# hellosunking/Microcket

Measured on AMD Instinct MI355X. Metric: read-pairs/sec through sam2pairs+dedup (150 bp PE, hg38 names, SAM text resident in HBM), higher is better.
Workload: dtype u8; 1 GPU; C2: 100 M 150 bp PE Micro-C read pairs, hg38, one MI355X -- 100000000 synthetic 150 bp PE read pairs per GPU, hg38 chromosome names, 1 lane(s), unc mode, sam=no, seed 20260105, one step = one pass over the whole resident data set + duplicate marking of the reported pairs on (chr1,pos1,chr2,pos2,strands) + per-chromosome-pair counts; preset=C2, pairs_per_gpu=100000001, sam_bytes_per_gpu=94584442002, block_groups=2097152, blocks=48, parallelism=shard1: independent read-group shards, no data-path collective

## Files before the change

microcket_amd/csrc/mkt_capi.cpp:

```cpp
#include "mkt_ctx.h"

extern "C" {

int mkt_abi_version(void) { return MKT_ABI_VERSION; }

const char* mkt_strerror(int code) {
    switch (code) {
    case MKT_OK: return "ok";
    case MKT_E_ARG: return "bad argument";
    case MKT_E_NO_DEVICE: return "no usable HIP device (this library has no CPU path)";
    case MKT_E_HIP: return "HIP runtime error";
    case MKT_E_NOMEM: return "out of memory";
    case MKT_E_CAPACITY: return "a QNAME group does not fit the block buffer";
    case MKT_E_KERNEL: return "kernel reported an internal error";
    case MKT_E_STATE: return "call order violated";
    case MKT_E_IO: return "temporary file error";
    case MKT_E_FORMAT: return "file refused";
    default: return "unknown error";
    }
}
const char* mkt_last_error(const mkt_ctx* ctx) { return ctx ? ctx->err.c_str() : g_create_error.c_str(); }

int mkt_device_count(void) {
    int n = 0;
// ... 67 lines not shown
    c->dims_probed = true;
    c->halo_widened = 0;
    if (c->cfg == CFG_SMALL || c->p.tiles != MKT_TILES_AUTO) return;
    c->dims = lean_dims(bytes_per_line);
    if (getenv("MKT_DEBUG_SYNC")) fprintf(stderr, "tile geometry: %.1f bytes per line -> tile %u, halos %u / %u\n", bytes_per_line, c->dims.tile, c->dims.hb, c->dims.hf);
}
static bool shrink_dims(mkt_ctx* c) {
    if (c->cfg == CFG_SMALL || c->dims.tile <= 2048u) return false;
    auto f = [](uint32_t x, uint32_t lo) { uint32_t y = ((uint32_t)(x * 0.6) + 15u) & ~15u; return y < lo ? lo : y; };
    c->dims.tile = f(c->dims.tile, 2048u); c->dims.hb = f(c->dims.hb, 256u); c->dims.hf = f(c->dims.hf, 512u);
    return true;
}
static bool widen_halos(mkt_ctx* c) {
    if (c->cfg == CFG_SMALL || c->halo_widened >= 2) return false;
    const TileDims mx = max_dims();
    auto f = [](uint32_t x, uint32_t hi) { uint32_t y = ((uint32_t)(x * 1.5) + 15u) & ~15u; return y > hi ? hi : y; };
    const uint32_t hb = f(c->dims.hb, mx.hb), hf = f(c->dims.hf, mx.hf);
    const uint32_t delta = (hb - c->dims.hb) + (hf - c->dims.hf);
    if (delta == 0 || c->dims.tile < delta + 2048u) return false;
    c->dims.tile -= delta; c->dims.hb = hb; c->dims.hf = hf;
    ++c->halo_widened;
    if (getenv("MKT_DEBUG_SYNC")) fprintf(stderr, "tile geometry: halos widened -> tile %u, halos %u / %u\n", c->dims.tile, c->dims.hb, c->dims.hf);
    return true;
}
static bool adapt_geometry(mkt_ctx* c, const BlockResult& r) {
    if (c->p.tiles != MKT_TILES_AUTO || c->p.ordered) return false;
    if (r.tiles >= 1000 && (uint64_t)r.pad2 * 500 > r.tiles && widen_halos(c)) return true;
    if (r.tiles >= 8 && (uint64_t)(r.pad - r.pad2) * 8 > r.tiles) return shrink_dims(c);
    return false;
}
static double probe_device_lines(mkt_ctx* c, const uint8_t* d_text, size_t n) {
    const size_t look = n < ((size_t)1 << 20) ? n : ((size_t)1 << 20);
    if (!look) return 0;
    if (!c->h_probe && (c->d_probe.alloc(1) != hipSuccess || c->h_probe.alloc(1) != hipSuccess)) return 0;
    if (hipMemsetAsync(c->d_probe, 0, sizeof(unsigned long long), c->stream) != hipSuccess) return 0;
    if (launch_count_newlines(d_text, look, c->d_probe, c->stream) != hipSuccess) return 0;
    if (hipMemcpyAsync(c->h_probe, c->d_probe, sizeof(unsigned long long), hipMemcpyDeviceToHost, c->stream) != hipSuccess) return 0;
    if (hipStreamSynchronize(c->stream) != hipSuccess) return 0;
    return *c->h_probe ? (double)look / (double)*c->h_probe : (double)look;
}
static void smaller_geometry(mkt_ctx* c, const uint8_t* d_text, size_t n) {
    if (c->cfg != CFG_SMALL && d_text) {
        const double avg = probe_device_lines(c, d_text, n);
        const TileDims d = avg > 0 ? lean_dims(avg) : c->dims;
        if (d.tile < c->dims.tile) { c->dims = d; return; }
    }
    if (!shrink_dims(c)) { c->cfg = CFG_SMALL; c->dims = small_dims(); }
}

struct StreamOut { uint8_t* gp; size_t gp_cap; uint8_t* gs; size_t gs_cap; hipEvent_t k0, k1, done; };
static int enqueue_block(mkt_ctx* c, const uint8_t* d_text, size_t n, int cfg, const TileDims& dims, size_t slot, const StreamOut* so = nullptr) {
    if (((uintptr_t)d_text & 15u) != 0) return fail(c, MKT_E_ARG, "block text must be 16-byte aligned");
    if (n >= kMaxBlock) return fail(c, MKT_E_ARG, "block of %zu bytes: must be < 2 GiB - 64 KiB", n);
    const uint32_t ntiles = num_tiles((uint32_t)n, dims.tile);
    BlockWs ws{nullptr, ntiles};
    const size_t ws_bytes = ws.bytes();
    int rc = ensure(c, c->d_ws, ws_bytes, ws_bytes + ws_bytes / 4, true);
    if (rc) return rc;
    ws.base = c->d_ws;
    if ((ntiles + finish_chunk_tiles() - 1) / finish_chunk_tiles() > BlockWs::kScanWords) return fail(c, MKT_E_ARG, "block has too many tiles for the finish scan");
    if ((rc = ensure_dev(c, c->d_pairs, n / 3 + 65536))) return rc;
    if (c->P.write_sam && (rc = ensure_dev(c, c->d_sam, n + n / 4 + 65536))) return rc;
    if (!c->d_sc && (rc = ensure_sc_list(c, 1))) return rc;
    KArgs a;
    memset(&a, 0, sizeof a);
    a.text = d_text; a.n = (uint32_t)n; a.ntiles = ntiles; a.dims = dims; a.P = c->P;
    a.descA = ws.descA(); a.descB = ws.descB(); a.descC = ws.descC();
    a.tile_last = ws.tile_last(); a.tile_groups = ws.tile_groups(); a.defer_list = ws.defer_list();
    a.cur = ws.cur();
    a.ticket = ws.ticket(); a.defer_count = ws.defer_count(); a.fast_ticket = ws.fast_ticket();
    a.last_tile = ws.last_tile(); a.scan_ticket = ws.scan_ticket(); a.scan_desc = ws.scan_desc();
    a.res = ws.res();
    a.ordered = c->p.ordered ? 1 : 0;
    a.run = c->d_run;
    a.nregions = c->p.ordered ? 1 : kMaxRegions;
    const size_t sc_need = (size_t)a.nregions * ((n / 256 / (size_t)a.nregions) * 2 + 1024);
    if ((rc = ensure(c, c->d_sc_tmp, sc_need, sc_need, true))) return rc;
    a.pairs_rcap = (c->d_pairs.cap() / a.nregions) & ~(uint64_t)15;
    a.sam_rcap = c->P.write_sam ? ((c->d_sam.cap() / a.nregions) & ~(uint64_t)15) : 0;
    a.sc_rcap = c->d_sc_tmp.cap() / a.nregions;
    a.out.pairs = c->d_pairs; a.out.pairs_cap = c->d_pairs.cap();
    a.out.sam = c->d_sam; a.out.sam_cap = c->P.write_sam ? c->d_sam.cap() : 0;
    a.out.sc = c->d_sc_tmp; a.out.sc_cap = c->d_sc_tmp.cap();
    a.sc_list = c->d_sc; a.sc_list_cap = c->d_sc.cap();
    if (c->p.extensions & MKT_EXT_KEYS) {
        if (!c->d_chr) { HIPCHK(c, c->d_chr.alloc(1)); HIPCHK(c, hipMemsetAsync(c->d_chr, 0, sizeof(ChrTab), c->stream)); }
        const size_t per = (n / 64 / (size_t)a.nregions) * 2 + 4096, need = per * a.nregions;
        if ((rc = ensure(c, c->d_keys_raw, need, need, true))) return rc;
        const double per_byte = c->key_density > 0 ? (c->key_density * 2 < 1.0 / 64 ? c->key_density * 2 : 1.0 / 64) : 1.0 / 64;
        const size_t want = (size_t)c->acc.emitted + (size_t)((double)(c->bytes_unsynced + n) * per_byte) + 65536;
        if (!c->d_key_list.fits(want)) {
            size_t ncap = c->d_key_list.cap() ? c->d_key_list.cap() * 2 : ((size_t)1 << 22);
            while (ncap < want) ncap *= 2;
            HIPCHK(c, hipStreamSynchronize(c->stream));
            HIPCHK(c, c->d_key_list.regrow_keep(ncap, c->d_key_list.cap()));
        }
        a.keys_rcap = c->d_keys_raw.cap() / a.nregions;
        a.out.keys = c->d_keys_raw; a.out.keys_cap = c->d_keys_raw.cap(); a.out.chr = c->d_chr;
        a.out.key_lanes = (c->p.extensions & MKT_EXT_LANES) ? 1u : 0u;
        a.key_list = c->d_key_list; a.key_list_cap = c->d_key_list.cap();
    }
#if defined(MKT_STAMPS)
    if (!c->d_stamps) { HIPCHK(c, c->d_stamps.alloc(kStampWords)); HIPCHK(c, hipMemset(c->d_stamps, 0, kStampWords * sizeof(unsigned long long))); }
    a.stamps = getenv("MKT_NO_STAMPS") ? nullptr : c->d_stamps;
    { const char* e = getenv("MKT_DEBUG_STOP"); a.debug_stop = e ? atoi(e) : 0; }
#endif
// ... 559 lines not shown
    int rc = mkt_sync(c);
    if (rc) return rc;
    const uint64_t K = total_groups ? total_groups : c->acc.groups;
    unsigned long long logged = 0;
    if (c->acc.sc) {
        if (!c->d_sc_logged) HIPCHK(c, c->d_sc_logged.alloc(1));
        HIPCHK(c, hipMemsetAsync(c->d_sc_logged, 0, sizeof(unsigned long long), c->stream));
        const uint64_t drop_group = c->acc.drops(drop_last != 0) ? c->acc.groups - 1 : ~0ull;
        HIPCHK(c, launch_sc_logged(c->d_sc, c->acc.sc, drop_group, group_offset, K, (uint32_t)c->p.ref_threads, c->d_sc_logged, c->stream));
        HIPCHK(c, hipMemcpyAsync(&logged, c->d_sc_logged, sizeof logged, hipMemcpyDeviceToHost, c->stream));
        HIPCHK(c, hipStreamSynchronize(c->stream));
    }
    RunStats s = c->acc.finish_logged(drop_last != 0, logged);
    memset(st, 0, sizeof *st);
    st->lowMap = s.counters[C_LOWMAP]; st->manyHits = s.counters[C_MANYHITS]; st->unpaired = s.counters[C_UNPAIRED];
    st->selfCircle = s.counters[C_SELFCIRCLE]; st->trans = s.counters[C_TRANS];
    st->cis10K = s.counters[C_CIS10K]; st->cis1K = s.counters[C_CIS1K]; st->cis0 = s.counters[C_CIS0];
    st->selfCircle_all = s.selfcircle_all;
    st->groups = s.groups; st->pairs = s.pairs; st->pair_bytes = s.pair_bytes; st->sam_bytes = s.sam_bytes;
    st->bytes_in = c->bytes_in; st->blocks = c->blocks;
    {
        std::lock_guard<std::mutex> g(c->mu);
        if (!c->finished) {
            if (!drop_last && (!c->tail_pairs.empty() || !c->tail_sam.empty())) {
                mkt_ctx::Chunk t;
                t.own_pairs.swap(c->tail_pairs); t.own_sam.swap(c->tail_sam);
                c->ready.push_back(std::move(t));
            }
            c->tail_pairs.clear(); c->tail_sam.clear();
            c->finished = true;
        }
    }
    c->cv.notify_all();
    return MKT_OK;
}

int mkt_reset(mkt_ctx* c) {
    if (!c) return MKT_E_ARG;
    HIPCHK(c, hipSetDevice(c->p.device));
    {
        std::unique_lock<std::mutex> lk(c->mu);
        c->cv.wait(lk, [&] { return c->async_rc != MKT_OK || c->jobs.empty(); });
        (void)sync_all(c);
        c->jobs.clear(); c->ready.clear(); c->handed = mkt_ctx::Chunk(); c->handed_valid = false;
        for (int i = 0; i < mkt_ctx::kIn; ++i) c->in[i].busy = false;
        for (int i = 0; i < mkt_ctx::kOut; ++i) { c->outs[i].dev_busy = false; c->outs[i].host_busy = false; }
        c->async_rc = MKT_OK; c->cur = 0; c->seq = 0; c->consumer_async = false;
    }
    HIPCHK(c, hipStreamSynchronize(c->stream));
    fold_timing(c);
    HIPCHK(c, hipMemsetAsync(c->d_run, 0, sizeof(DevRun), c->stream));
    HIPCHK(c, hipStreamSynchronize(c->stream));
    c->acc = RunAccum();
    c->sc_unfolded = 0; c->bytes_unsynced = 0; c->emitted_unfolded = 0;
    c->sc_density = 0; c->key_density = 0; c->probing = true;
    c->dims_probed = c->p.tiles != MKT_TILES_AUTO || c->p.ordered || c->cfg == CFG_SMALL;
    if (c->d_chr) HIPCHK(c, hipMemsetAsync(c->d_chr, 0, sizeof(ChrTab), c->stream));
    c->res_used = c->res_folded = 0;
    c->h_len = 0;
    c->tail_pairs.clear(); c->tail_sam.clear(); c->drained_pairs.clear(); c->drained_sam.clear();
    c->input_done = c->finished = false;
    c->bytes_in = 0; c->blocks = 0;
    return MKT_OK;
}

int mkt_format_log(const mkt_stats* st, char* out, size_t cap) {
    if (!st || !out) return MKT_E_ARG;
    return snprintf(out, cap, "lowMap\t%u\nmanyHits\t%u\nunpaired\t%u\nselfCircle\t%u\ntrans\t%u\ncis10K\t%u\ncis1K\t%u\ncis0\t%u\n",
                    st->lowMap, st->manyHits, st->unpaired, st->selfCircle, st->trans, st->cis10K, st->cis1K, st->cis0);
}

int mkt_get_timing(const mkt_ctx* c, mkt_timing* t) {
    if (!c || !t) return MKT_E_ARG;
    t->tile_kernel_ms = c->folded_ms; t->tile_launches = c->folded_launches; t->tile_bytes = c->folded_bytes; t->other_ms = 0;
    t->tiles = c->tiles_total; t->deferred_tiles = c->tiles_deferred;
    return MKT_OK;
}
int mkt_reset_timing(mkt_ctx* c) {
    if (!c) return MKT_E_ARG;
    c->folded_ms = 0; c->folded_launches = 0; c->folded_bytes = 0; c->tiles_total = 0; c->tiles_deferred = 0;
    std::lock_guard<std::mutex> g(c->mu);
    c->replays = mkt_replays{0, 0, 0, 0, 0};
    return MKT_OK;
}
int mkt_get_replays(const mkt_ctx* c, mkt_replays* r) {
    if (!c || !r) return MKT_E_ARG;
    std::lock_guard<std::mutex> g(const_cast<mkt_ctx*>(c)->mu);
    *r = c->replays;
    return MKT_OK;
}

}
```

microcket_amd/csrc/mkt_capi_ext.cpp:

```cpp
#include "mkt_ctx.h"

extern "C" {

static int ensure_dedup_work(mkt_ctx* c, uint64_t n);
int mkt_ext_dedup(mkt_ctx* c, int drop_last, uint64_t* total, uint64_t* dups, uint8_t* flags, size_t flags_cap) {
    if (!c) return MKT_E_ARG;
    if (!(c->p.extensions & MKT_EXT_KEYS)) return fail(c, MKT_E_STATE, "context created without MKT_EXT_KEYS");
    int rc = mkt_sync(c);
    if (rc) return rc;
    const uint64_t n = ext_key_count(c, drop_last);
    if (total) *total = n;
    if (dups) *dups = 0;
    if (n == 0) return MKT_OK;
    if (flags && flags_cap < n) return fail(c, MKT_E_ARG, "flags buffer too small (%llu needed)", (unsigned long long)n);
    const size_t wb = dedup_work_bytes(n);
    if ((rc = ensure_dedup_work(c, n))) return rc;
    HIPCHK(c, launch_dedup(c->d_key_list, n, c->d_dd_flags, c->d_dd_work.get(), wb, c->d_dd_res, c->stream));
    HIPCHK(c, hipMemcpyAsync(c->h_dd_res, c->d_dd_res, sizeof(DedupResult), hipMemcpyDeviceToHost, c->stream));
    if (flags) HIPCHK(c, hipMemcpyAsync(flags, c->d_dd_flags, n, hipMemcpyDeviceToHost, c->stream));
    HIPCHK(c, hipStreamSynchronize(c->stream));
    if (dups) *dups = c->h_dd_res->dups;
    return MKT_OK;
}
int mkt_ext_chr_names(mkt_ctx* c, char* out, size_t cap, size_t* len) {
    if (!c || !len) return MKT_E_ARG;
    if (!(c->p.extensions & MKT_EXT_KEYS)) return fail(c, MKT_E_STATE, "context created without MKT_EXT_KEYS");
    int rc = mkt_sync(c);
    if (rc) return rc;
    *len = 0;
    if (!c->d_chr) return MKT_OK;
    std::vector<unsigned long long> hh(kChrSlots);
    std::vector<uint8_t> names((size_t)kChrSlots * 64);
    HIPCHK(c, hipMemcpy(hh.data(), c->d_chr->hash, kChrSlots * sizeof(unsigned long long), hipMemcpyDeviceToHost));
    HIPCHK(c, hipMemcpy(names.data(), c->d_chr->name, names.size(), hipMemcpyDeviceToHost));
    std::string txt;
    char num[16];
    for (uint32_t s2 = 0; s2 < kChrSlots; ++s2) if (hh[s2]) {
        snprintf(num, sizeof num, "%u", s2);
        txt += num; txt += '\t'; txt.append((const char*)&names[(size_t)s2 * 64], names[(size_t)s2 * 64 + 63]); txt += '\n';
    }
    *len = txt.size();
    if (out) { if (cap < txt.size()) return fail(c, MKT_E_ARG, "buffer too small (%zu needed)", txt.size()); memcpy(out, txt.data(), txt.size()); }
    return MKT_OK;
}
int mkt_ext_keys_fetch(mkt_ctx* c, int drop_last, void* keys, size_t cap_bytes, uint64_t* n) {
    if (!c || !n) return MKT_E_ARG;
    if (!(c->p.extensions & MKT_EXT_KEYS)) return fail(c, MKT_E_STATE, "context created without MKT_EXT_KEYS");
    int rc = mkt_sync(c);
    if (rc) return rc;
    *n = ext_key_count(c, drop_last);
    if (keys && *n) {
        if (cap_bytes < *n * sizeof(KeyRec)) return fail(c, MKT_E_ARG, "key buffer too small (%llu bytes needed)", (unsigned long long)(*n * sizeof(KeyRec)));
        HIPCHK(c, hipMemcpy(keys, c->d_key_list, (size_t)*n * sizeof(KeyRec), hipMemcpyDeviceToHost));
    }
    return MKT_OK;
}
static int ensure_dedup_work(mkt_ctx* c, uint64_t n) {
    const size_t wb = dedup_work_bytes(n);
    int rc;
    if ((rc = ensure(c, c->d_dd_flags, n, n + n / 8 + 4096, false))) return rc;
    if ((rc = ensure(c, c->d_dd_work, wb, wb + wb / 8, false))) return rc;
    if (!c->h_dd_res) { HIPCHK(c, c->d_dd_res.alloc(1)); HIPCHK(c, c->h_dd_res.alloc(1)); }
    return MKT_OK;
}
int mkt_ext_dedup_device(mkt_ctx* c, const void* d_keys, uint64_t n, uint8_t* d_flags, uint64_t* dups) {
    if (!c || (n && (!d_keys || !d_flags))) return MKT_E_ARG;
    HIPCHK(c, hipSetDevice(c->p.device));
    if (dups) *dups = 0;
    if (n == 0) return MKT_OK;
    int rc = ensure_dedup_work(c, n);
    if (rc) return rc;
    HIPCHK(c, launch_dedup((const KeyRec*)d_keys, n, d_flags, c->d_dd_work.get(), dedup_work_bytes(n), c->d_dd_res, c->stream));
    HIPCHK(c, hipMemcpyAsync(c->h_dd_res, c->d_dd_res, sizeof(DedupResult), hipMemcpyDeviceToHost, c->stream));
    HIPCHK(c, hipStreamSynchronize(c->stream));
// ... 129 lines not shown
                    const hipError_t e = hipDeviceEnablePeerAccess(cs[b]->p.device, 0);
                    if (e != hipSuccess) (void)hipGetLastError();
                }
            }
    for (uint32_t r = 0; r < world; ++r) {
        mkt_ctx* c = cs[r];
        HIPCHK(c, hipSetDevice(c->p.device));
        sd[r].nrecv = 0;
        for (uint32_t s2 = 0; s2 < world; ++s2) sd[r].nrecv += sd[s2].cnt[r];
        if (!sd[r].nrecv) continue;
        HIPCHK(c, sd[r].d_recv.alloc((size_t)sd[r].nrecv * sizeof(KeyRec)));
        HIPCHK(c, sd[r].d_flags.alloc((size_t)sd[r].nrecv));
        uint64_t at = 0;
        for (uint32_t s2 = 0; s2 < world; ++s2) {
            uint64_t soff = 0;
            for (uint32_t d = 0; d < r; ++d) soff += sd[s2].cnt[d];
            const uint64_t k = sd[s2].cnt[r];
            if (k) HIPCHK(c, hipMemcpyPeerAsync(sd[r].d_recv + at * sizeof(KeyRec), c->p.device, sd[s2].d_send + soff * sizeof(KeyRec), cs[s2]->p.device, (size_t)k * sizeof(KeyRec), c->stream));
            at += k;
        }
    }
    uint64_t all_dups = 0;
    for (uint32_t r = 0; r < world; ++r) {
        mkt_ctx* c = cs[r];
        HIPCHK(c, hipSetDevice(c->p.device));
        HIPCHK(c, hipStreamSynchronize(c->stream));
        uint64_t d = 0;
        const int rc = mkt_ext_dedup_device(c, sd[r].d_recv, sd[r].nrecv, sd[r].d_flags, &d);
        if (rc) return rc;
        all_dups += d;
    }
    for (uint32_t s2 = 0; s2 < world; ++s2) {
        mkt_ctx* c = cs[s2];
        HIPCHK(c, hipSetDevice(c->p.device));
        if (!sd[s2].n) { dups[s2] = 0; continue; }
        HIPCHK(c, sd[s2].d_back.alloc((size_t)sd[s2].n));
        uint64_t soff = 0;
        for (uint32_t r = 0; r < world; ++r) {
            uint64_t roff = 0;
            for (uint32_t q = 0; q < s2; ++q) roff += sd[q].cnt[r];
            const uint64_t k = sd[s2].cnt[r];
            if (k) HIPCHK(c, hipMemcpyPeerAsync(sd[s2].d_back + soff, c->p.device, sd[r].d_flags + roff, cs[r]->p.device, (size_t)k, c->stream));
            soff += k;
        }
        HIPCHK(c, hipStreamSynchronize(c->stream));
        const int rc = mkt_ext_unpartition(c, sd[s2].d_back, flags ? flags[s2] : nullptr, flags_cap ? flags_cap[s2] : 0, &dups[s2]);
        if (rc) return rc;
    }
    uint64_t sum = 0;
    for (uint32_t r = 0; r < world; ++r) sum += dups[r];
    if (sum != all_dups) return fail(c0, MKT_E_KERNEL, "duplicate counts disagree after the exchange (%llu marked, %llu returned)", (unsigned long long)all_dups, (unsigned long long)sum);
    return MKT_OK;
}
int mkt_ext_chrstat(mkt_ctx* c, int drop_last, char* out, size_t cap, size_t* len) {
    if (!c || !len) return MKT_E_ARG;
    if (!(c->p.extensions & MKT_EXT_KEYS)) return fail(c, MKT_E_STATE, "context created without MKT_EXT_KEYS");
    int rc = mkt_sync(c);
    if (rc) return rc;
    *len = 0;
    const uint64_t n = ext_key_count(c, drop_last);
    if (n == 0 || !c->d_chr) return MKT_OK;
    const size_t name_bytes = (size_t)kChrSlots * 64, hash_bytes = kChrSlots * sizeof(unsigned long long);
    if (!c->h_chr_stage) HIPCHK(c, c->h_chr_stage.alloc(hash_bytes + name_bytes + kChrSlots * sizeof(uint16_t)));
    unsigned long long* hh = (unsigned long long*)c->h_chr_stage.get();
    uint8_t* names = c->h_chr_stage + hash_bytes;
    uint16_t* dense = (uint16_t*)(c->h_chr_stage + hash_bytes + name_bytes);
    HIPCHK(c, hipMemcpyAsync(hh, c->d_chr->hash, hash_bytes, hipMemcpyDeviceToHost, c->stream));
    HIPCHK(c, hipMemcpyAsync(names, c->d_chr->name, name_bytes, hipMemcpyDeviceToHost, c->stream));
    HIPCHK(c, hipStreamSynchronize(c->stream));
    std::vector<std::pair<std::string, uint32_t>> used;
    for (uint32_t s2 = 0; s2 < kChrSlots; ++s2) if (hh[s2]) used.emplace_back(std::string((const char*)&names[(size_t)s2 * 64], names[(size_t)s2 * 64 + 63]), s2);
    std::sort(used.begin(), used.end());
    const uint32_t nd = (uint32_t)used.size();
    memset(dense, 0, kChrSlots * sizeof(uint16_t));
    for (uint32_t d = 0; d < nd; ++d) dense[used[d].second] = (uint16_t)d;
    const size_t cells = (size_t)nd * nd, cnt_bytes = cells * sizeof(unsigned long long);
    if (!c->d_dense) HIPCHK(c, c->d_dense.alloc(kChrSlots));
    if ((rc = ensure(c, c->d_chr_counts, cells, cells, false)) || (rc = ensure(c, c->h_chr_counts, cells, cells, false))) return rc;
    HIPCHK(c, hipMemcpyAsync(c->d_dense, dense, kChrSlots * sizeof(uint16_t), hipMemcpyHostToDevice, c->stream));
    HIPCHK(c, hipMemsetAsync(c->d_chr_counts, 0, cnt_bytes, c->stream));
    HIPCHK(c, launch_chrstat(c->d_key_list, n, c->d_dense, nd, c->d_chr_counts, c->stream));
    HIPCHK(c, hipMemcpyAsync(c->h_chr_counts, c->d_chr_counts, cnt_bytes, hipMemcpyDeviceToHost, c->stream));
    HIPCHK(c, hipStreamSynchronize(c->stream));
    const unsigned long long* counts = c->h_chr_counts;
    std::string txt;
    char num[32];
    for (uint32_t a2 = 0; a2 < nd; ++a2)
        for (uint32_t b2 = 0; b2 < nd; ++b2)
            if (counts[(size_t)a2 * nd + b2]) {
                snprintf(num, sizeof num, "%llu", counts[(size_t)a2 * nd + b2]);
                txt += used[a2].first; txt += '\t'; txt += used[b2].first; txt += '\t'; txt += num; txt += '\n';
            }
    *len = txt.size();
    if (out) { if (cap < txt.size()) return fail(c, MKT_E_ARG, "chrstat buffer too small (%zu needed)", txt.size()); memcpy(out, txt.data(), txt.size()); }
    return MKT_OK;
}

}
```

microcket_amd/csrc/mkt_ctx.h:

```cpp
#pragma once
#include <hip/hip_runtime.h>
#include <stdarg.h>
#include <stdio.h>
#include <stdlib.h>
#include <string.h>
#include <algorithm>
#include <string>
#include <utility>
#include <chrono>
#include <condition_variable>
#include <deque>
#include <mutex>
#include <thread>
#include <vector>

#include "../../include/mkt.h"
#include "mkt_launch.h"
#include "mkt_devbuf.h"

using namespace mkt;

static const size_t kMaxBlock = ((size_t)1 << 31) - 65536;
static const uint32_t kFastRoundsDefault = 8;
static const size_t kStampWords = 20;

inline thread_local std::string g_create_error;

struct mkt_ctx {
    mkt_params p;
    Params P;
    DevStream stream, s_in, s_out;
    int cfg = CFG_FAST;
    TileDims dims = {0, 0, 0};
    bool dims_probed = false;
    DevBuf<unsigned long long> d_probe; PinBuf<unsigned long long> h_probe;
    TileDims last_dims = {0, 0, 0};
    const uint8_t* last_text = nullptr;
    bool probing = true;
    size_t block_cap = 0;
    GrowBuf<uint8_t> d_pairs, d_sam;
    GrowBuf<uint64_t> d_sc;
    DevBuf<unsigned long long> d_sc_logged;
    PinBuf<uint8_t> h_chr_stage; DevBuf<uint16_t> d_dense;
    GrowBuf<uint8_t> d_dd_flags, d_dd_work;
    DevBuf<DedupResult> d_dd_res; PinBuf<DedupResult> h_dd_res;
    GrowBuf<uint32_t> d_perm; DevBuf<uint32_t> d_part_hist; DevBuf<uint16_t> d_lut; uint64_t part_n = 0;
    GrowBuf<unsigned long long> d_chr_counts; PinGrowBuf<unsigned long long> h_chr_counts;
    double sc_density = 0;
    GrowBuf<uint64_t> d_sc_tmp;
    GrowBuf<KeyRec> d_keys_raw;
    GrowBuf<KeyRec> d_key_list;
    DevBuf<ChrTab> d_chr;
    GrowBuf<uint8_t> d_ws;
    DevBuf<DevRun> d_run;
    size_t h_len = 0;
    PinBuf<BlockResult> h_res; size_t res_slots = 0, res_used = 0, res_folded = 0;
    std::vector<DevBuf<uint8_t>> uploads;
    std::vector<const uint8_t*> res_text; std::vector<size_t> res_n;
    static constexpr int kIn = 3, kOut = 2;
    static constexpr size_t kHead = 65536;
    enum { EV_H2D, EV_K0, EV_K1, EV_DONE };
    struct InSlot { PinBuf<uint8_t> h; DevBuf<uint8_t> d; bool busy = false; DevEvents<4> ev; };
    struct OutSlot { GrowBuf<uint8_t> d_pairs, d_sam; PinGrowBuf<uint8_t> h; bool dev_busy = false, host_busy = false; };
    struct Job { int in_slot, out_slot; size_t n; int cfg; TileDims dims; int attempts; };
    struct Chunk { const char* pairs = nullptr; size_t pairs_len = 0; const char* sam = nullptr; size_t sam_len = 0; int out_slot = -1;
                   std::vector<char> own_pairs, own_sam; };
    InSlot in[kIn];
    OutSlot outs[kOut];
    std::deque<Job> jobs;
    std::deque<Chunk> ready;
    Chunk handed; bool handed_valid = false;
    std::mutex mu;
    std::condition_variable cv;
    std::thread worker;
    bool worker_started = false, stop = false;
    int async_rc = MKT_OK;
    bool consumer_async = false;
    int cur = 0;
    uint64_t seq = 0;
    std::vector<char> tail_pairs, tail_sam, drained_pairs, drained_sam;
    RunAccum acc;
    bool input_done = false, finished = false;
    uint64_t bytes_in = 0, blocks = 0;
    size_t last_n = 0;
    double key_density = 0;
    uint64_t emitted_unfolded = 0;
    uint64_t sc_unfolded = 0;
    uint64_t bytes_unsynced = 0;
    struct Timed { DevEvents<2> ev; uint64_t bytes = 0; };
    std::deque<Timed> ev;
    double folded_ms = 0; uint64_t folded_launches = 0, folded_bytes = 0;
    uint64_t tiles_total = 0, tiles_deferred = 0;
    mkt_replays replays = {0, 0, 0, 0, 0};
    GrowBuf<char> d_syn;
    GrowBuf<uint64_t> d_syn_sizes;
    DevBuf<unsigned long long> d_stamps;
    uint32_t fast_rounds = kFastRoundsDefault;
    bool no_lean = false;
    int halo_widened = 0;
    std::string err;
// ... 36 lines not shown
```

microcket_amd/csrc/mkt_kernels.hip:

```cpp
#include <hip/hip_runtime.h>
#include <type_traits>
#include "mkt_launch.h"

namespace mkt {

constexpr int NT = 256;
constexpr uint64_t FLAG_AGG = 1ull << 62, FLAG_PREFIX = 2ull << 62, PAYLOAD = (1ull << 62) - 1;
constexpr uint32_t LOOKBACK_SPIN_LIMIT = 1u << 22;

struct ScanScratch { uint64_t a[NT / 64], b[NT / 64]; };

#if defined(MKT_STAMPS)
#define STAMP_DECL() unsigned long long stamp_prev_ = 0, stamp_first_ = 0, stamp_acc_[16] = {0, 0, 0, 0, 0, 0, 0, 0, 0, 0, 0, 0, 0, 0, 0, 0}
#define STAMP(k)                                                                        \
    do {                                                                                \
        if (tid == 0 && a.stamps) {                                                     \
            const unsigned long long now_ = __builtin_amdgcn_s_memtime();               \
            if ((k) > 0) stamp_acc_[(k)] += now_ - stamp_prev_;                         \
            else if (!stamp_first_) stamp_first_ = __builtin_amdgcn_s_memrealtime();   \
            stamp_prev_ = now_;                                                         \
        }                                                                               \
    } while (0)
#define STAMP_SPAN(t0_)                                                                 \
    do {                                                                                \
// ... 1026 lines not shown

uint32_t fast_max_workgroups(int) { return 256u * 4u; }

hipError_t launch_tiles(const KArgs& a, int cfg, int grid, hipStream_t s) {
    if (a.ntiles == 0) return hipSuccess;
    if (!dims_ok(a.dims, cfg == CFG_SMALL ? small_dims() : max_dims())) return hipErrorInvalidValue;
    if (cfg == CFG_SMALL) hipLaunchKernelGGL(k_tiles<CfgSmall>, dim3(grid), dim3(NT), 0, s, a);
    else hipLaunchKernelGGL(k_tiles<CfgFast>, dim3(grid), dim3(NT), 0, s, a);
    return hipGetLastError();
}
hipError_t launch_fast(const KArgs& a, int, int grid, hipStream_t s) {
    if (a.ntiles == 0) return hipSuccess;
    if (!dims_ok(a.dims, max_dims())) return hipErrorInvalidValue;
    hipLaunchKernelGGL((k_fast<CfgLean, NT, 2, 4>), dim3(grid), dim3(NT), 0, s, a);
    return hipGetLastError();
}
__global__ void k_count_nl(const uint8_t* text, size_t n, unsigned long long* out) {
    unsigned long long mine = 0;
    const size_t nv = n >> 4;
    for (size_t v = (size_t)blockIdx.x * blockDim.x + threadIdx.x; v < nv; v += (size_t)gridDim.x * blockDim.x) {
        const uint4 x = reinterpret_cast<const uint4*>(text)[v];
        mine += __popc(nl_flags(x.x)) + __popc(nl_flags(x.y)) + __popc(nl_flags(x.z)) + __popc(nl_flags(x.w));
    }
    if (blockIdx.x == 0 && threadIdx.x == 0) for (size_t b = nv << 4; b < n; ++b) mine += text[b] == '\n';
    for (int d = 32; d >= 1; d >>= 1) mine += shfl_xor64(mine, d);
    if ((threadIdx.x & 63) == 0 && mine) atomicAdd(out, mine);
}
hipError_t launch_count_newlines(const uint8_t* text, size_t n, unsigned long long* out, hipStream_t s) {
    if (n) hipLaunchKernelGGL(k_count_nl, dim3(64), dim3(256), 0, s, text, n, out);
    return hipGetLastError();
}
hipError_t launch_finish(const KArgs& a, hipStream_t s) {
    const unsigned chunks = (a.ntiles + NTF - 1) / NTF;
    if (chunks) hipLaunchKernelGGL(k_finish_scan, dim3(chunks), dim3(NTF), 0, s, a);
    hipLaunchKernelGGL(k_finish, dim3(kFinishGrid), dim3(NTF), 0, s, a);
    if (a.keys_rcap) hipLaunchKernelGGL(k_keys_place, dim3(2048), dim3(256), 0, s, a);
    hipLaunchKernelGGL(k_run_advance, dim3(1), dim3(64), 0, s, a);
    return hipGetLastError();
}
uint32_t finish_chunk_tiles() { return NTF; }

constexpr int DD_WG = 256;
constexpr int DS_WG = 512;
constexpr int DS_NW = DS_WG / 64;
constexpr int DS_T = 8192;
constexpr int DS_K = DS_T / DS_WG;
constexpr int DS_D = 7, DS_R = 1 << DS_D;
constexpr int DS_SCAN_WG = 1024, DS_SCAN_V = 8;
constexpr uint64_t kKeyMask1 = 0xFFFFFFFFC000FFFFull;
static_assert(DS_R == 2 * 64, "the scatter's prologue gives each lane of wave 0 two digits");

__device__ inline bool key_eq(const KeyRec& x, const KeyRec& y) { return x.k0 == y.k0 && (x.k1 & kKeyMask1) == (y.k1 & kKeyMask1); }

__global__ __launch_bounds__(DS_WG) void k_dd_prep(const KeyRec* keys, uint64_t n, int ib, uint64_t* rec, uint32_t* cnt, uint32_t G) {
    __shared__ uint32_t c[DS_R];
    if (threadIdx.x < DS_R) c[threadIdx.x] = 0;
    __syncthreads();
    const uint64_t b = (uint64_t)blockIdx.x * DS_T, e = b + DS_T < n ? b + DS_T : n, hi = ~((1ull << ib) - 1ull);
    for (uint64_t j = b + threadIdx.x; j < e; j += DS_WG) {
        const uint64_t r = (mix64(keys[j].k0 ^ mix64(keys[j].k1 & kKeyMask1)) & hi) | j;
        rec[j] = r;
        atomicAdd(&c[(r >> ib) & (DS_R - 1)], 1u);
    }
    __syncthreads();
    if (threadIdx.x < DS_R) cnt[threadIdx.x * G + blockIdx.x] = c[threadIdx.x];
}
__global__ __launch_bounds__(DS_WG) void k_dd_count(const uint64_t* rec, uint64_t n, int shift, uint32_t* cnt, uint32_t G) {
    __shared__ uint32_t c[DS_R];
    if (threadIdx.x < DS_R) c[threadIdx.x] = 0;
    __syncthreads();
    const uint64_t b = (uint64_t)blockIdx.x * DS_T, m = (b + DS_T < n ? b + DS_T : n) - b;
    const ulonglong2* v = reinterpret_cast<const ulonglong2*>(rec + b);
    for (uint64_t i = threadIdx.x; i < m / 2; i += DS_WG) {
        const ulonglong2 x = v[i];
        atomicAdd(&c[(x.x >> shift) & (DS_R - 1)], 1u);
        atomicAdd(&c[(x.y >> shift) & (DS_R - 1)], 1u);
    }
    if ((m & 1) && threadIdx.x == 0) atomicAdd(&c[(rec[b + m - 1] >> shift) & (DS_R - 1)], 1u);
    __syncthreads();
    if (threadIdx.x < DS_R) cnt[threadIdx.x * G + blockIdx.x] = c[threadIdx.x];
}
__global__ __launch_bounds__(DS_SCAN_WG) void k_dd_dscan(uint32_t* cnt, uint32_t G, uint32_t* tot) {
    __shared__ uint32_t wsum[DS_SCAN_WG / 64];
    const int lane = threadIdx.x & 63, wv = threadIdx.x >> 6;
    uint32_t* row = cnt + (uint64_t)blockIdx.x * G;
    uint32_t carry = 0;
    for (uint32_t base = 0; base < G; base += DS_SCAN_WG * DS_SCAN_V) {
        const uint32_t i0 = base + threadIdx.x * DS_SCAN_V;
        uint32_t v[DS_SCAN_V], s = 0;
#pragma unroll
        for (int k = 0; k < DS_SCAN_V; ++k) { v[k] = i0 + k < G ? row[i0 + k] : 0u; s += v[k]; }
        const uint32_t inc = wave_iscan32(s);
        if (lane == 63) wsum[wv] = inc;
        __syncthreads();
        uint32_t pre = carry, all = 0;
#pragma unroll
        for (int w = 0; w < DS_SCAN_WG / 64; ++w) { const uint32_t x = wsum[w]; if (w < wv) pre += x; all += x; }
        pre += inc - s;
#pragma unroll
        for (int k = 0; k < DS_SCAN_V; ++k) { if (i0 + k < G) row[i0 + k] = pre; pre += v[k]; }
        carry += all;
        __syncthreads();
    }
    if (threadIdx.x == 0) tot[blockIdx.x] = carry;
}
__global__ __launch_bounds__(DS_WG, 4) void k_dd_scatter(const uint64_t* rec, uint64_t n, int shift, const uint32_t* cnt, const uint32_t* tot, uint32_t G, uint64_t* rec2) {
    __shared__ uint64_t tile[DS_T];
    __shared__ uint32_t wrun[DS_NW][DS_R];
    __shared__ uint32_t gdelta[DS_R];
    const int tid = threadIdx.x, lane = tid & 63, wv = tid >> 6;
    const uint64_t b = (uint64_t)blockIdx.x * DS_T, m = (b + DS_T < n ? b + DS_T : n) - b;
    uint32_t gc0 = 0, gc1 = 0, t0 = 0, t1 = 0;
    if (wv == 0) {
        gc0 = cnt[(uint64_t)(2 * lane) * G + blockIdx.x]; gc1 = cnt[(uint64_t)(2 * lane + 1) * G + blockIdx.x];
        t0 = tot[2 * lane]; t1 = tot[2 * lane + 1];
    }
    for (int i = tid; i < DS_NW * DS_R; i += DS_WG) (&wrun[0][0])[i] = 0u;
    __syncthreads();
// ... 38 lines not shown
    __syncthreads();
#pragma unroll
    for (int k = 0; k < DS_K; ++k) {
        const uint64_t i = (uint64_t)wv * (DS_T / DS_NW) + k * 64 + lane;
        if (i < m) tile[wrun[wv][(uint32_t)(r[k] >> shift) & (DS_R - 1)] + ((loc[k / 2] >> (16 * (k & 1))) & 0xFFFFu)] = r[k];
    }
    __syncthreads();
    for (uint32_t i = tid; i < m; i += DS_WG) {
        const uint64_t x = tile[i];
        rec2[gdelta[(uint32_t)(x >> shift) & (DS_R - 1)] + i] = x;
    }
}
__global__ __launch_bounds__(NT) void k_dd_scan(uint32_t* hist, uint32_t m) {
    __shared__ ScanScratch sc;
    __shared__ uint64_t carry;
    if (threadIdx.x == 0) carry = 0;
    __syncthreads();
    for (uint32_t base = 0; base < m; base += NT) {
        const uint32_t i = base + threadIdx.x;
        uint64_t x = i < m ? hist[i] : 0, d = 0, tx, td, e = x;
        block_exscan2(e, d, tx, td, sc);
        if (i < m) hist[i] = (uint32_t)(carry + e);
        __syncthreads();
        if (threadIdx.x == 0) carry += tx;
        __syncthreads();
    }
}
__global__ __launch_bounds__(256) void k_dd_mark(const KeyRec* keys, const uint64_t* rec, uint64_t n, int ib, uint64_t run_mask, uint8_t* flags, DedupResult* res) {
    const uint64_t imask = (1ull << ib) - 1ull, j = (uint64_t)blockIdx.x * blockDim.x + threadIdx.x;
    bool dup = false;
    if (j < n) {
        const uint64_t r = rec[j];
        uint64_t o = j ? rec[j - 1] : ~r;
        bool have = false;
        KeyRec me;
        for (uint64_t b = j - 1; !((o ^ r) & run_mask);) {
            if (!((o ^ r) >> ib)) {
                if (!have) { me = keys[r & imask]; have = true; }
                if (key_eq(keys[o & imask], me)) { dup = true; break; }
            }
            if (b-- == 0) break;
            o = rec[b];
        }
        if (dup) flags[r & imask] = 1;
    }
    const uint64_t m = __ballot(dup);
    if ((threadIdx.x & 63) == 0 && m) atomicAdd((unsigned long long*)&res->dups, (unsigned long long)__popcll(m));
    if (blockIdx.x == 0 && threadIdx.x == 0) res->total = n;
}
size_t dedup_work_bytes(uint64_t n) {
    const uint64_t G = (n + DS_T - 1) / DS_T;
    return (size_t)(n * (8 + 8) + DS_R * (G + 1) * 4 + 4096);
}
hipError_t launch_dedup(const KeyRec* keys, uint64_t n, uint8_t* flags, void* work, size_t work_bytes, DedupResult* d_res, hipStream_t s) {
    hipError_t e = hipMemsetAsync(d_res, 0, sizeof(DedupResult), s);
    if (e != hipSuccess || n == 0) return e;
    if (work_bytes < dedup_work_bytes(n) || n >= (1ull << 32)) return hipErrorInvalidValue;
    const uint32_t G = (uint32_t)((n + DS_T - 1) / DS_T);
    uint8_t* w = (uint8_t*)(((uintptr_t)work + 255) & ~(uintptr_t)255);
    uint64_t* rA = (uint64_t*)w; w += ((n * 8 + 255) & ~255ull);
    uint64_t* rB = (uint64_t*)w; w += ((n * 8 + 255) & ~255ull);
    uint32_t* cnt = (uint32_t*)w;
    uint32_t* tot = cnt + (uint64_t)DS_R * G;
    int ib = 1;
    while ((1ull << ib) < n) ++ib;
    int bits = 2;
    while (bits < 34 && (1ull << (bits - 2)) < n) ++bits;
    bits = bits < 12 ? 12 : (bits > 32 ? 32 : bits);
    const int passes = (bits + DS_D - 1) / DS_D;
    const int sorted = passes * DS_D < 64 - ib ? passes * DS_D : 64 - ib;
    hipLaunchKernelGGL(k_dd_prep, dim3(G), dim3(DS_WG), 0, s, keys, n, ib, rA, cnt, G);
    for (int p = 0; p < passes; ++p) {
        if (p) hipLaunchKernelGGL(k_dd_count, dim3(G), dim3(DS_WG), 0, s, (const uint64_t*)rA, n, ib + DS_D * p, cnt, G);
        hipLaunchKernelGGL(k_dd_dscan, dim3(DS_R), dim3(DS_SCAN_WG), 0, s, cnt, G, tot);
        hipLaunchKernelGGL(k_dd_scatter, dim3(G), dim3(DS_WG), 0, s, (const uint64_t*)rA, n, ib + DS_D * p, (const uint32_t*)cnt, (const uint32_t*)tot, G, rB);
        uint64_t* t = rA; rA = rB; rB = t;
    }
    const uint64_t run_mask = ((1ull << sorted) - 1ull) << ib;
    e = hipMemsetAsync(flags, 0, n, s);
    if (e != hipSuccess) return e;
    hipLaunchKernelGGL(k_dd_mark, dim3((unsigned)((n + 255) / 256)), dim3(256), 0, s, keys, (const uint64_t*)rA, n, ib, run_mask, flags, d_res);
    return hipGetLastError();
}
size_t radix64_count_bytes(uint64_t n) { return (size_t)(DS_R * ((n + DS_T - 1) / DS_T + 1) * 4 + 4096); }
hipError_t launch_radix64(uint64_t*& rA, uint64_t*& rB, uint64_t n, int lo_bit, int nbits, uint32_t* cnt, hipStream_t s) {
    if (n == 0 || nbits <= 0) return hipSuccess;
    if (n >= (1ull << 32) || lo_bit < 0 || lo_bit + nbits > 64) return hipErrorInvalidValue;
    const uint32_t G = (uint32_t)((n + DS_T - 1) / DS_T);
    uint32_t* tot = cnt + (uint64_t)DS_R * G;
    for (int sh = lo_bit; sh < lo_bit + nbits; sh += DS_D) {
        hipLaunchKernelGGL(k_dd_count, dim3(G), dim3(DS_WG), 0, s, (const uint64_t*)rA, n, sh, cnt, G);
        hipLaunchKernelGGL(k_dd_dscan, dim3(DS_R), dim3(DS_SCAN_WG), 0, s, cnt, G, tot);
        hipLaunchKernelGGL(k_dd_scatter, dim3(G), dim3(DS_WG), 0, s, (const uint64_t*)rA, n, sh, (const uint32_t*)cnt, (const uint32_t*)tot, G, rB);
        uint64_t* t = rA; rA = rB; rB = t;
    }
    return hipGetLastError();
}

constexpr uint32_t kMaxWorld = 16;
__device__ inline KeyRec part_remap(KeyRec r, const uint16_t* lut) {
    if (lut) {
        const uint64_t a = lut[(r.k0 >> 45) & (kChrSlots - 1u)], b = lut[(r.k0 >> 32) & (kChrSlots - 1u)];
        r.k0 = (a << 45) | (b << 32) | (r.k0 & 0xFFFFFFFFull);
    }
    return r;
}
__device__ inline uint32_t part_dest(const KeyRec& r, uint32_t world) { return (uint32_t)(mix64(r.k0 ^ mix64(r.k1 & kKeyMask1)) % world); }
__global__ __launch_bounds__(DD_WG) void k_part_hist(const KeyRec* keys, uint64_t n, uint64_t per, const uint16_t* lut, uint32_t world, uint32_t* hist, uint32_t G) {
    __shared__ uint32_t cnt[kMaxWorld];
    if (threadIdx.x < kMaxWorld) cnt[threadIdx.x] = 0;
    __syncthreads();
    const uint64_t b = (uint64_t)blockIdx.x * per, e = b + per < n ? b + per : n;
    for (uint64_t j = b + threadIdx.x; j < e; j += DD_WG) atomicAdd(&cnt[part_dest(part_remap(keys[j], lut), world)], 1u);
    __syncthreads();
    if (threadIdx.x < kMaxWorld) hist[threadIdx.x * G + blockIdx.x] = cnt[threadIdx.x];
}
__global__ __launch_bounds__(DD_WG) void k_part_scatter(const KeyRec* keys, uint64_t n, uint64_t per, const uint16_t* lut, uint32_t world, const uint32_t* hist,
                                                       uint32_t G, KeyRec* send, uint32_t* perm) {
    __shared__ uint32_t base[kMaxWorld];
    __shared__ uint32_t wcnt[DD_WG / 64][kMaxWorld];
    const int tid = threadIdx.x, lane = tid & 63, wv = tid >> 6;
    if (tid < (int)kMaxWorld) base[tid] = hist[tid * G + blockIdx.x];
    __syncthreads();
    const uint64_t b = (uint64_t)blockIdx.x * per, e = b + per < n ? b + per : n;
// ... 175 lines not shown
```

microcket_amd/csrc/mkt_launch.h:

```cpp
#pragma once
#include <hip/hip_runtime.h>
#include "mkt_host.h"
#include "mkt_fast.h"
#include "mkt_synth.h"

namespace mkt {

enum { CFG_FAST = 0, CFG_SMALL = 1 };

struct DevRun { uint64_t groups, sc, emitted; };

struct alignas(128) RegionCur { unsigned long long a, b; unsigned long long pad[14]; };
constexpr int kMaxRegions = 16;
constexpr int kCurShift = 36;
constexpr unsigned long long kCurLow = (1ull << kCurShift) - 1ull;

constexpr uint32_t kFastAllStatic = 0xFFFFFFFFu;
struct KArgs {
    const uint8_t* text;
    uint32_t n;
    uint32_t ntiles;
    TileDims dims;
    uint32_t fast_dyn0;
    Params P;
// ... 13 lines not shown
    int32_t use_list;
    BlockResult* res;
    DevRun* run;
    RegionCur* cur;
    int32_t nregions;
    uint64_t pairs_rcap, sam_rcap, sc_rcap;
    uint64_t* sc_list;
    uint64_t sc_list_cap;
    uint64_t keys_rcap;
    KeyRec* key_list;
    uint64_t key_list_cap;
    OutPtrs out;
    unsigned long long* stamps;
    int32_t debug_stop;
};

struct BlockWs {
    uint8_t* base;
    uint32_t ntiles;
    static constexpr size_t kScanWords = 1024;
    size_t tiles_bytes() const { return ((size_t)ntiles * (3 * sizeof(uint64_t) + sizeof(TileLast) + sizeof(uint64_t) + sizeof(uint32_t)) + 127) & ~(size_t)127; }
    size_t bytes() const { return tiles_bytes() + kMaxRegions * sizeof(RegionCur) + 256 + kScanWords * sizeof(uint64_t) + sizeof(BlockResult); }
    uint64_t* descA() const { return (uint64_t*)base; }
    uint64_t* descB() const { return descA() + ntiles; }
    uint64_t* descC() const { return descB() + ntiles; }
    TileLast* tile_last() const { return (TileLast*)(descC() + ntiles); }
    uint64_t* tile_groups() const { return (uint64_t*)(tile_last() + ntiles); }
    uint32_t* defer_list() const { return (uint32_t*)(tile_groups() + ntiles); }
    RegionCur* cur() const { return (RegionCur*)(base + tiles_bytes()); }
    uint8_t* counters() const { return (uint8_t*)(cur() + kMaxRegions); }
    uint32_t* ticket() const { return (uint32_t*)counters(); }
    uint32_t* defer_count() const { return (uint32_t*)(counters() + 64); }
    uint32_t* defer_ticket() const { return (uint32_t*)(counters() + 128); }
    uint32_t* fast_ticket() const { return (uint32_t*)(counters() + 160); }
    int* last_tile() const { return (int*)(counters() + 192); }
    uint32_t* scan_ticket() const { return (uint32_t*)(counters() + 224); }
    uint64_t* scan_desc() const { return (uint64_t*)(counters() + 256); }
    BlockResult* res() const { return (BlockResult*)(scan_desc() + kScanWords); }
};

TileDims small_dims();
TileDims max_dims();
uint32_t fast_max_workgroups(int cfg);
hipError_t launch_count_newlines(const uint8_t* text, size_t n, unsigned long long* out, hipStream_t s);
hipError_t launch_tiles(const KArgs& a, int cfg, int grid, hipStream_t s);
hipError_t launch_fast(const KArgs& a, int cfg, int grid, hipStream_t s);
uint32_t finish_chunk_tiles();
hipError_t launch_finish(const KArgs& a, hipStream_t s);
hipError_t launch_gather(const BlockResult* d_res, const uint8_t* src, uint64_t rcap, uint8_t* dst, uint64_t dst_cap, int which, uint64_t max_bytes, hipStream_t s);
hipError_t launch_sc_logged(const uint64_t* list, uint64_t n, uint64_t drop_group, uint64_t group_offset, uint64_t K_total, uint32_t ref_threads,
                            unsigned long long* out, hipStream_t s);

struct DedupResult { uint64_t total, dups; };
hipError_t launch_dedup(const KeyRec* keys, uint64_t n, uint8_t* flags, void* work, size_t work_bytes, DedupResult* d_res, hipStream_t s);
size_t dedup_work_bytes(uint64_t n);
size_t radix64_count_bytes(uint64_t n);
hipError_t launch_radix64(uint64_t*& rA, uint64_t*& rB, uint64_t n, int lo_bit, int nbits, uint32_t* cnt, hipStream_t s);
size_t partition_work_bytes();
hipError_t launch_partition(const KeyRec* keys, uint64_t n, const uint16_t* d_lut, uint32_t world, uint32_t* hist, KeyRec* send, uint32_t* perm, uint32_t* G_out, hipStream_t s);
hipError_t launch_unpermute(const uint8_t* in, const uint32_t* perm, uint64_t n, uint8_t* out, unsigned long long* dups, hipStream_t s);
hipError_t launch_chrstat(const KeyRec* keys, uint64_t n, const uint16_t* dense_of_slot, uint32_t ndense, unsigned long long* counts, hipStream_t s);

hipError_t launch_synth_sizes(const SynParams& p, uint64_t first, uint64_t n, uint64_t* sizes, hipStream_t s);
hipError_t launch_exscan(uint64_t* v, uint64_t n, uint64_t* total, hipStream_t s);
hipError_t launch_synth_write(const SynParams& p, uint64_t first, uint64_t n, const uint64_t* offs, char* out, hipStream_t s);
hipError_t launch_synth_tail(const SynParams& p, char* out, hipStream_t s);
size_t synth_tail_bytes(const SynParams& p);

}
```

Before: 2.339 billion read-pairs/s.

## Fuse per-chromosome-pair counting into dedup prep kernel and stash results

The chromosome-pair count histogram is now computed inside the dedup prep kernel, which already reads every key. Counts go to a shared-memory 32x32 table, with global atomics as the fallback. The result is stashed on the host and validated by a generation counter, key count and emitted count, so the later chrstat call skips its own pass over the keys and its separate kernel launch. The trade-off is a grid-stride prep kernel capped at 2048 workgroups, an extra host sync for the dense map before dedup, and stash invalidation logic that must stay correct.

```diff
diff --git a/microcket_amd/csrc/mkt_capi.cpp b/microcket_amd/csrc/mkt_capi.cpp
--- a/microcket_amd/csrc/mkt_capi.cpp
+++ b/microcket_amd/csrc/mkt_capi.cpp
@@ -143,6 +143,7 @@
 static int enqueue_block(mkt_ctx* c, const uint8_t* d_text, size_t n, int cfg, const TileDims& dims, size_t slot, const StreamOut* so = nullptr) {
     if (((uintptr_t)d_text & 15u) != 0) return fail(c, MKT_E_ARG, "block text must be 16-byte aligned");
     if (n >= kMaxBlock) return fail(c, MKT_E_ARG, "block of %zu bytes: must be < 2 GiB - 64 KiB", n);
+    ++c->key_gen;
     const uint32_t ntiles = num_tiles((uint32_t)n, dims.tile);
     BlockWs ws{nullptr, ntiles};
     const size_t ws_bytes = ws.bytes();
@@ -808,6 +809,7 @@
     HIPCHK(c, hipMemsetAsync(c->d_run, 0, sizeof(DevRun), c->stream));
     HIPCHK(c, hipStreamSynchronize(c->stream));
     c->acc = RunAccum();
+    ++c->key_gen; c->chr_stash.valid = false;
     c->sc_unfolded = 0; c->bytes_unsynced = 0; c->emitted_unfolded = 0;
     c->sc_density = 0; c->key_density = 0; c->probing = true;
     c->dims_probed = c->p.tiles != MKT_TILES_AUTO || c->p.ordered || c->cfg == CFG_SMALL;
diff --git a/microcket_amd/csrc/mkt_capi_ext.cpp b/microcket_amd/csrc/mkt_capi_ext.cpp
--- a/microcket_amd/csrc/mkt_capi_ext.cpp
+++ b/microcket_amd/csrc/mkt_capi_ext.cpp
@@ -3,6 +3,8 @@
 extern "C" {
 
 static int ensure_dedup_work(mkt_ctx* c, uint64_t n);
+typedef std::vector<std::pair<std::string, uint32_t>> ChrNames;
+static int chr_dense_map(mkt_ctx* c, ChrNames& used);
 int mkt_ext_dedup(mkt_ctx* c, int drop_last, uint64_t* total, uint64_t* dups, uint8_t* flags, size_t flags_cap) {
     if (!c) return MKT_E_ARG;
     if (!(c->p.extensions & MKT_EXT_KEYS)) return fail(c, MKT_E_STATE, "context created without MKT_EXT_KEYS");
@@ -15,11 +17,23 @@
     if (flags && flags_cap < n) return fail(c, MKT_E_ARG, "flags buffer too small (%llu needed)", (unsigned long long)n);
     const size_t wb = dedup_work_bytes(n);
     if ((rc = ensure_dedup_work(c, n))) return rc;
-    HIPCHK(c, launch_dedup(c->d_key_list, n, c->d_dd_flags, c->d_dd_work.get(), wb, c->d_dd_res, c->stream));
+    mkt_ctx::ChrStash& st = c->chr_stash;
+    st.valid = false;
+    st.used.clear();
+    if (c->d_chr && (rc = chr_dense_map(c, st.used))) return rc;
+    const uint32_t nd = (uint32_t)st.used.size();
+    const size_t cnt_bytes = (size_t)nd * nd * sizeof(unsigned long long);
+    HIPCHK(c, launch_dedup(c->d_key_list, n, c->d_dd_flags, c->d_dd_work.get(), wb, c->d_dd_res, c->stream,
+                           nd ? c->d_dense.get() : nullptr, nd, nd ? c->d_chr_counts.get() : nullptr));
     HIPCHK(c, hipMemcpyAsync(c->h_dd_res, c->d_dd_res, sizeof(DedupResult), hipMemcpyDeviceToHost, c->stream));
+    if (nd) HIPCHK(c, hipMemcpyAsync(c->h_chr_counts, c->d_chr_counts, cnt_bytes, hipMemcpyDeviceToHost, c->stream));
     if (flags) HIPCHK(c, hipMemcpyAsync(flags, c->d_dd_flags, n, hipMemcpyDeviceToHost, c->stream));
     HIPCHK(c, hipStreamSynchronize(c->stream));
     if (dups) *dups = c->h_dd_res->dups;
+    if (nd) {
+        st.counts.assign(c->h_chr_counts.get(), c->h_chr_counts.get() + (size_t)nd * nd);
+        st.n = n; st.emitted = c->acc.emitted; st.gen = c->key_gen; st.valid = true;
+    }
     return MKT_OK;
 }
 int mkt_ext_chr_names(mkt_ctx* c, char* out, size_t cap, size_t* len) {
@@ -255,14 +269,7 @@
     if (sum != all_dups) return fail(c0, MKT_E_KERNEL, "duplicate counts disagree after the exchange (%llu marked, %llu returned)", (unsigned long long)all_dups, (unsigned long long)sum);
     return MKT_OK;
 }
-int mkt_ext_chrstat(mkt_ctx* c, int drop_last, char* out, size_t cap, size_t* len) {
-    if (!c || !len) return MKT_E_ARG;
-    if (!(c->p.extensions & MKT_EXT_KEYS)) return fail(c, MKT_E_STATE, "context created without MKT_EXT_KEYS");
-    int rc = mkt_sync(c);
-    if (rc) return rc;
-    *len = 0;
-    const uint64_t n = ext_key_count(c, drop_last);
-    if (n == 0 || !c->d_chr) return MKT_OK;
+static int chr_dense_map(mkt_ctx* c, ChrNames& used) {
     const size_t name_bytes = (size_t)kChrSlots * 64, hash_bytes = kChrSlots * sizeof(unsigned long long);
     if (!c->h_chr_stage) HIPCHK(c, c->h_chr_stage.alloc(hash_bytes + name_bytes + kChrSlots * sizeof(uint16_t)));
     unsigned long long* hh = (unsigned long long*)c->h_chr_stage.get();
@@ -271,21 +278,43 @@
     HIPCHK(c, hipMemcpyAsync(hh, c->d_chr->hash, hash_bytes, hipMemcpyDeviceToHost, c->stream));
     HIPCHK(c, hipMemcpyAsync(names, c->d_chr->name, name_bytes, hipMemcpyDeviceToHost, c->stream));
     HIPCHK(c, hipStreamSynchronize(c->stream));
-    std::vector<std::pair<std::string, uint32_t>> used;
+    used.clear();
     for (uint32_t s2 = 0; s2 < kChrSlots; ++s2) if (hh[s2]) used.emplace_back(std::string((const char*)&names[(size_t)s2 * 64], names[(size_t)s2 * 64 + 63]), s2);
     std::sort(used.begin(), used.end());
     const uint32_t nd = (uint32_t)used.size();
+    if (nd == 0) return MKT_OK;
     memset(dense, 0, kChrSlots * sizeof(uint16_t));
     for (uint32_t d = 0; d < nd; ++d) dense[used[d].second] = (uint16_t)d;
-    const size_t cells = (size_t)nd * nd, cnt_bytes = cells * sizeof(unsigned long long);
+    const size_t cells = (size_t)nd * nd;
+    int rc;
     if (!c->d_dense) HIPCHK(c, c->d_dense.alloc(kChrSlots));
     if ((rc = ensure(c, c->d_chr_counts, cells, cells, false)) || (rc = ensure(c, c->h_chr_counts, cells, cells, false))) return rc;
     HIPCHK(c, hipMemcpyAsync(c->d_dense, dense, kChrSlots * sizeof(uint16_t), hipMemcpyHostToDevice, c->stream));
-    HIPCHK(c, hipMemsetAsync(c->d_chr_counts, 0, cnt_bytes, c->stream));
-    HIPCHK(c, launch_chrstat(c->d_key_list, n, c->d_dense, nd, c->d_chr_counts, c->stream));
-    HIPCHK(c, hipMemcpyAsync(c->h_chr_counts, c->d_chr_counts, cnt_bytes, hipMemcpyDeviceToHost, c->stream));
-    HIPCHK(c, hipStreamSynchronize(c->stream));
-    const unsigned long long* counts = c->h_chr_counts;
+    HIPCHK(c, hipMemsetAsync(c->d_chr_counts, 0, cells * sizeof(unsigned long long), c->stream));
+    return MKT_OK;
+}
+int mkt_ext_chrstat(mkt_ctx* c, int drop_last, char* out, size_t cap, size_t* len) {
+    if (!c || !len) return MKT_E_ARG;
+    if (!(c->p.extensions & MKT_EXT_KEYS)) return fail(c, MKT_E_STATE, "context created without MKT_EXT_KEYS");
+    int rc = mkt_sync(c);
+    if (rc) return rc;
+    *len = 0;
+    const uint64_t n = ext_key_count(c, drop_last);
+    if (n == 0 || !c->d_chr) return MKT_OK;
+    const mkt_ctx::ChrStash& st = c->chr_stash;
+    const bool stashed = st.valid && st.n == n && st.emitted == c->acc.emitted && st.gen == c->key_gen;
+    ChrNames mapped;
+    if (!stashed) {
+        if ((rc = chr_dense_map(c, mapped))) return rc;
+        const uint32_t nd0 = (uint32_t)mapped.size();
+        if (nd0 == 0) return MKT_OK;
+        HIPCHK(c, launch_chrstat(c->d_key_list, n, c->d_dense, nd0, c->d_chr_counts, c->stream));
+        HIPCHK(c, hipMemcpyAsync(c->h_chr_counts, c->d_chr_counts, (size_t)nd0 * nd0 * sizeof(unsigned long long), hipMemcpyDeviceToHost, c->stream));
+        HIPCHK(c, hipStreamSynchronize(c->stream));
+    }
+    const ChrNames& used = stashed ? st.used : mapped;
+    const unsigned long long* counts = stashed ? st.counts.data() : c->h_chr_counts.get();
+    const uint32_t nd = (uint32_t)used.size();
     std::string txt;
     char num[32];
     for (uint32_t a2 = 0; a2 < nd; ++a2)
diff --git a/microcket_amd/csrc/mkt_ctx.h b/microcket_amd/csrc/mkt_ctx.h
--- a/microcket_amd/csrc/mkt_ctx.h
+++ b/microcket_amd/csrc/mkt_ctx.h
@@ -46,6 +46,13 @@
     DevBuf<DedupResult> d_dd_res; PinBuf<DedupResult> h_dd_res;
     GrowBuf<uint32_t> d_perm; DevBuf<uint32_t> d_part_hist; DevBuf<uint16_t> d_lut; uint64_t part_n = 0;
     GrowBuf<unsigned long long> d_chr_counts; PinGrowBuf<unsigned long long> h_chr_counts;
+    struct ChrStash {
+        bool valid = false;
+        uint64_t n = 0, emitted = 0, gen = 0;
+        std::vector<std::pair<std::string, uint32_t>> used;
+        std::vector<unsigned long long> counts;
+    } chr_stash;
+    uint64_t key_gen = 0;
     double sc_density = 0;
     GrowBuf<uint64_t> d_sc_tmp;
     GrowBuf<KeyRec> d_keys_raw;
diff --git a/microcket_amd/csrc/mkt_kernels.hip b/microcket_amd/csrc/mkt_kernels.hip
--- a/microcket_amd/csrc/mkt_kernels.hip
+++ b/microcket_amd/csrc/mkt_kernels.hip
@@ -1102,18 +1102,39 @@
 
 __device__ inline bool key_eq(const KeyRec& x, const KeyRec& y) { return x.k0 == y.k0 && (x.k1 & kKeyMask1) == (y.k1 & kKeyMask1); }
 
-__global__ __launch_bounds__(DS_WG) void k_dd_prep(const KeyRec* keys, uint64_t n, int ib, uint64_t* rec, uint32_t* cnt, uint32_t G) {
+constexpr uint32_t kPrepChrGrid = 2048;
+template <bool CHR>
+__global__ __launch_bounds__(DS_WG) void k_dd_prep(const KeyRec* keys, uint64_t n, int ib, uint64_t* rec, uint32_t* cnt, uint32_t G,
+                                                   const uint16_t* dense_of_slot, uint32_t ndense, unsigned long long* chr_counts) {
     __shared__ uint32_t c[DS_R];
-    if (threadIdx.x < DS_R) c[threadIdx.x] = 0;
-    __syncthreads();
-    const uint64_t b = (uint64_t)blockIdx.x * DS_T, e = b + DS_T < n ? b + DS_T : n, hi = ~((1ull << ib) - 1ull);
-    for (uint64_t j = b + threadIdx.x; j < e; j += DS_WG) {
-        const uint64_t r = (mix64(keys[j].k0 ^ mix64(keys[j].k1 & kKeyMask1)) & hi) | j;
-        rec[j] = r;
-        atomicAdd(&c[(r >> ib) & (DS_R - 1)], 1u);
-    }
-    __syncthreads();
-    if (threadIdx.x < DS_R) cnt[threadIdx.x * G + blockIdx.x] = c[threadIdx.x];
+    __shared__ uint32_t loc[CHR ? 32 * 32 : 1];
+    if (CHR) for (int k = threadIdx.x; k < 1024; k += DS_WG) loc[k] = 0;
+    const uint64_t hi = ~((1ull << ib) - 1ull);
+    for (uint32_t t = blockIdx.x; t < G; t += gridDim.x) {
+        if (threadIdx.x < DS_R) c[threadIdx.x] = 0;
+        __syncthreads();
+        const uint64_t b = (uint64_t)t * DS_T, e = b + DS_T < n ? b + DS_T : n;
+        for (uint64_t j = b + threadIdx.x; j < e; j += DS_WG) {
+            const uint64_t k0 = keys[j].k0;
+            const uint64_t r = (mix64(k0 ^ mix64(keys[j].k1 & kKeyMask1)) & hi) | j;
+            rec[j] = r;
+            atomicAdd(&c[(r >> ib) & (DS_R - 1)], 1u);
+            if (CHR) {
+                const uint32_t ca = dense_of_slot[(k0 >> 45) & (kChrSlots - 1u)], cb = dense_of_slot[(k0 >> 32) & (kChrSlots - 1u)];
+                if (ca < 32u && cb < 32u) atomicAdd(&loc[ca * 32u + cb], 1u);
+                else if (ca < ndense && cb < ndense) atomicAdd(&chr_counts[(uint64_t)ca * ndense + cb], 1ull);
+            }
+        }
+        __syncthreads();
+        if (threadIdx.x < DS_R) cnt[threadIdx.x * G + t] = c[threadIdx.x];
+    }
+    if (CHR) {
+        __syncthreads();
+        for (int k = threadIdx.x; k < 1024; k += DS_WG) {
+            const uint32_t ca = k >> 5, cb = k & 31;
+            if (loc[k] && ca < ndense && cb < ndense) atomicAdd(&chr_counts[(uint64_t)ca * ndense + cb], (unsigned long long)loc[k]);
+        }
+    }
 }
 __global__ __launch_bounds__(DS_WG) void k_dd_count(const uint64_t* rec, uint64_t n, int shift, uint32_t* cnt, uint32_t G) {
     __shared__ uint32_t c[DS_R];
@@ -1258,7 +1279,8 @@
     const uint64_t G = (n + DS_T - 1) / DS_T;
     return (size_t)(n * (8 + 8) + DS_R * (G + 1) * 4 + 4096);
 }
-hipError_t launch_dedup(const KeyRec* keys, uint64_t n, uint8_t* flags, void* work, size_t work_bytes, DedupResult* d_res, hipStream_t s) {
+hipError_t launch_dedup(const KeyRec* keys, uint64_t n, uint8_t* flags, void* work, size_t work_bytes, DedupResult* d_res, hipStream_t s,
+                        const uint16_t* dense_of_slot, uint32_t ndense, unsigned long long* chr_counts) {
     hipError_t e = hipMemsetAsync(d_res, 0, sizeof(DedupResult), s);
     if (e != hipSuccess || n == 0) return e;
     if (work_bytes < dedup_work_bytes(n) || n >= (1ull << 32)) return hipErrorInvalidValue;
@@ -1275,7 +1297,10 @@
     bits = bits < 12 ? 12 : (bits > 32 ? 32 : bits);
     const int passes = (bits + DS_D - 1) / DS_D;
     const int sorted = passes * DS_D < 64 - ib ? passes * DS_D : 64 - ib;
-    hipLaunchKernelGGL(k_dd_prep, dim3(G), dim3(DS_WG), 0, s, keys, n, ib, rA, cnt, G);
+    if (chr_counts && dense_of_slot && ndense)
+        hipLaunchKernelGGL(k_dd_prep<true>, dim3(G < kPrepChrGrid ? G : kPrepChrGrid), dim3(DS_WG), 0, s, keys, n, ib, rA, cnt, G, dense_of_slot, ndense, chr_counts);
+    else
+        hipLaunchKernelGGL(k_dd_prep<false>, dim3(G), dim3(DS_WG), 0, s, keys, n, ib, rA, cnt, G, (const uint16_t*)nullptr, 0u, (unsigned long long*)nullptr);
     for (int p = 0; p < passes; ++p) {
         if (p) hipLaunchKernelGGL(k_dd_count, dim3(G), dim3(DS_WG), 0, s, (const uint64_t*)rA, n, ib + DS_D * p, cnt, G);
         hipLaunchKernelGGL(k_dd_dscan, dim3(DS_R), dim3(DS_SCAN_WG), 0, s, cnt, G, tot);
diff --git a/microcket_amd/csrc/mkt_launch.h b/microcket_amd/csrc/mkt_launch.h
--- a/microcket_amd/csrc/mkt_launch.h
+++ b/microcket_amd/csrc/mkt_launch.h
@@ -89,7 +89,8 @@
                             unsigned long long* out, hipStream_t s);
 
 struct DedupResult { uint64_t total, dups; };
-hipError_t launch_dedup(const KeyRec* keys, uint64_t n, uint8_t* flags, void* work, size_t work_bytes, DedupResult* d_res, hipStream_t s);
+hipError_t launch_dedup(const KeyRec* keys, uint64_t n, uint8_t* flags, void* work, size_t work_bytes, DedupResult* d_res, hipStream_t s,
+                        const uint16_t* dense_of_slot = nullptr, uint32_t ndense = 0, unsigned long long* chr_counts = nullptr);
 size_t dedup_work_bytes(uint64_t n);
 size_t radix64_count_bytes(uint64_t n);
 hipError_t launch_radix64(uint64_t*& rA, uint64_t*& rB, uint64_t n, int lo_bit, int nbits, uint32_t* cnt, hipStream_t s);
```

Measured after the change: 2.345 billion read-pairs/s, median of 3. Within noise of the previous version (+0.3%).
